# raineyeh/Marching-Cube-for-Implicit-Surfaces

Measured on NVIDIA B200. Metric: Gvoxels/s, higher is better.
Workload: dtype f32

## Files before the change

marching-cube-for-implicit-surfaces_b200/csrc/mcb_api.cu:

```cuda
#include <cuda_runtime.h>
#include <dlfcn.h>

#include <algorithm>
#include <chrono>
#include <future>
#include <cmath>
#include <cstdio>
#include <cstring>
#include <map>
#include <mutex>
#include <new>
#include <string>
#include <vector>

#include "../../include/mcb.h"
#include "mcb_kernels.cuh"
#include "mcb_jit.h"
#include "mcb_lower.h"

using namespace mcbk;

namespace {

struct EqSlot {
// ... 49 lines not shown
    unsigned long long* d_amb = nullptr;
    uint32_t cap_amb = 0;
    size_t cap_tile_entries = 0;
    size_t cap_tiles = 0;
    unsigned long long* d_rec = nullptr;
    uint32_t* d_trioff = nullptr;
    unsigned long long cap_active = 0;
    float4* d_pos = nullptr;
    float4* d_nrm = nullptr;
    unsigned long long cap_tris = 0;
    bool nrm_allocated = false;
    int mesh_mode = MCB_MESH_SOUP;
    float* d_vlist = nullptr;
    float* d_vnrm = nullptr;
    uint32_t* d_tlist = nullptr;
    unsigned long long cap_verts = 0, cap_itris = 0;
    bool vnrm_allocated = false;
    float* h_out_v = nullptr;
    uint32_t* h_out_t = nullptr;
    float* h_out_n = nullptr;
    unsigned long long h_cap_v = 0, h_cap_t = 0;
    cudaStream_t copy_stream = nullptr;
    cudaEvent_t seg_ev[9] = {};
    cudaEvent_t fork_ev[2] = {};
    unsigned long long* d_bounds = nullptr;
    unsigned long long* h_bounds = nullptr;
    bool streamed = false;
    bool seed_on = false;
    int jit = MCB_JIT_AUTO;
    std::string jit_note;
    struct JitKernel { cudaLibrary_t lib = nullptr; cudaKernel_t kernel = nullptr, signs = nullptr, fill = nullptr; };
    const JitKernel* jit_cur = nullptr;
    std::map<std::string, JitKernel> jit_cache;
    struct JitBuilt { std::string err; std::vector<char> cubin; float ms = 0.f; };
    std::map<std::string, std::future<JitBuilt>> jit_pending;
    std::map<std::string, std::string> jit_failed;
    bool jit_sync = false;
    bool jit_used = false;
    float ms_compile = 0.f;
    bool repeat_on = false;
    float repeat_step = 0.f;
    uint32_t* d_cw = nullptr;
    size_t cap_cw = 0;
    float seed[3] = {0.f, 0.f, 0.f};
    void* nccl_comm = nullptr;
    int comm_rank = 0, comm_nranks = 1;
    cudaStream_t comm_stream = nullptr;
// ... 412 lines not shown
    return MCB_OK;
}

int mcb_create(int device, mcb_ctx** out) {
    if (!out) return MCB_E_ARG;
    *out = nullptr;
    int ndev = 0;
    if (cudaGetDeviceCount(&ndev) != cudaSuccess || ndev <= 0 || device < 0 || device >= ndev) return MCB_E_NODEVICE;
    mcb_ctx* ctx = new (std::nothrow) mcb_ctx();
    if (!ctx) return MCB_E_NOMEM;
    ctx->device = device;
    auto bail = [&](int code) { mcb_destroy(ctx); return code; };
    if (cudaSetDevice(device) != cudaSuccess) return bail(MCB_E_NODEVICE);
    cudaDeviceProp prop;
    if (cudaGetDeviceProperties(&prop, device) != cudaSuccess) return bail(MCB_E_NODEVICE);
    ctx->sm_count = prop.multiProcessorCount;
    if (cudaStreamCreateWithFlags(&ctx->own_stream, cudaStreamNonBlocking) != cudaSuccess) return bail(MCB_E_CUDA);
    ctx->stream = ctx->own_stream;
    for (auto& e : ctx->ev)
        if (cudaEventCreate(&e) != cudaSuccess) return bail(MCB_E_CUDA);
    if (cudaStreamCreateWithFlags(&ctx->copy_stream, cudaStreamNonBlocking) != cudaSuccess) return bail(MCB_E_CUDA);
    for (auto& e : ctx->seg_ev)
        if (cudaEventCreateWithFlags(&e, cudaEventDisableTiming) != cudaSuccess) return bail(MCB_E_CUDA);
    for (auto& e : ctx->fork_ev)
        if (cudaEventCreateWithFlags(&e, cudaEventDisableTiming) != cudaSuccess) return bail(MCB_E_CUDA);
    if (cudaMalloc((void**)&ctx->d_bounds, 3 * 9 * 8) != cudaSuccess) return bail(MCB_E_NOMEM);
    if (cudaMallocHost((void**)&ctx->h_bounds, 3 * 9 * 8) != cudaSuccess) return bail(MCB_E_NOMEM);
    if (cudaMalloc((void**)&ctx->d_ctr, sizeof(Counters)) != cudaSuccess) return bail(MCB_E_NOMEM);
    if (cudaMallocHost((void**)&ctx->h_ctr, sizeof(Counters)) != cudaSuccess) return bail(MCB_E_NOMEM);
    ClsTables tb;
    int8_t face[256];
    mcb_build_ambiguity_faces(face);
    for (int q = 0; q < 256; q++) {
        tb.tri[q] = MCB_TRI_WORDS[q];
        tb.face[q] = face[q];
        tb.ntri[q] = (uint8_t)mcb_tri_count(MCB_TRI_WORDS[q]);
        tb.emask[q] = 0;
        for (int e = 0; e < 12; e++) tb.emask[q] |= (uint16_t)((((q >> mcb_edge_a(e)) ^ (q >> mcb_edge_b(e))) & 1) << e);
    }
    if (cudaMalloc((void**)&ctx->d_cls, sizeof(ClsTables)) != cudaSuccess) return bail(MCB_E_NOMEM);
    if (cudaMemcpy(ctx->d_cls, &tb, sizeof tb, cudaMemcpyHostToDevice) != cudaSuccess) return bail(MCB_E_CUDA);
    {
        const int stack_bytes = MCB_MAX_STACK * kEvalRows * kEvalThreads * (int)sizeof(float);
        const void* evals[] = {(const void*)eval_field_kernel<true, true>, (const void*)eval_field_kernel<false, true>,
                               (const void*)eval_blocks_kernel<true>,      (const void*)eval_blocks_kernel<false>,
                               (const void*)eval_field_kernel<true, true, true>, (const void*)eval_blocks_kernel<true, true>};
        for (const void* k : evals)
            if (cudaFuncSetAttribute(k, cudaFuncAttributeMaxDynamicSharedMemorySize, stack_bytes) != cudaSuccess) return bail(MCB_E_CUDA);
// ... 10 lines not shown
    if (rc < 0) return bail(rc);
    *out = ctx;
    return MCB_OK;
}

void mcb_destroy(mcb_ctx* ctx) {
    if (!ctx) return;
    cudaSetDevice(ctx->device);
    if (ctx->stream) cudaStreamSynchronize(ctx->stream);
    for (auto& s : ctx->eq) free_slot(s);
    for (auto& kv : ctx->jit_cache) if (kv.second.lib) cudaLibraryUnload(kv.second.lib);
    cudaFree(ctx->d_fflags); cudaFree(ctx->d_flist); cudaFree(ctx->d_cw); cudaFree(ctx->d_bcls); cudaFree(ctx->d_elist); cudaFree(ctx->d_cand); cudaFree(ctx->d_scls); cudaFree(ctx->d_slist);
    cudaFree(ctx->d_bounds_iv); cudaFree(ctx->d_ent); cudaFree(ctx->d_tile_u32); cudaFree(ctx->d_amb);
    cudaFree(ctx->d_cs); cudaFree(ctx->d_F); cudaFree(ctx->d_S); cudaFree(ctx->d_V); cudaFree(ctx->d_tables);
    cudaFree(ctx->d_cls); cudaFree(ctx->d_ctr);
    if (ctx->h_ctr) cudaFreeHost(ctx->h_ctr);
    cudaFree(ctx->d_rec); cudaFree(ctx->d_trioff); cudaFree(ctx->d_pos); cudaFree(ctx->d_nrm);
    cudaFree(ctx->d_vlist); cudaFree(ctx->d_vnrm); cudaFree(ctx->d_tlist); cudaFree(ctx->d_item); cudaFree(ctx->d_vinfo);
    cudaFree(ctx->d_chunk_new); cudaFree(ctx->d_fn); cudaFree(ctx->d_nh_count); cudaFree(ctx->d_nh_start); cudaFree(ctx->d_nh_cursor);
    cudaFree(ctx->d_nh_sums); cudaFree(ctx->d_nh_adj);
    cudaFree(ctx->d_mark); cudaFree(ctx->d_changed); cudaFree(ctx->d_seed_u32); cudaFree(ctx->d_rec2); cudaFree(ctx->d_trioff2);
    for (auto& e : ctx->ev) if (e) cudaEventDestroy(e);
    for (auto& e : ctx->seg_ev) if (e) cudaEventDestroy(e);
    for (auto& e : ctx->fork_ev) if (e) cudaEventDestroy(e);
    if (ctx->copy_stream) cudaStreamDestroy(ctx->copy_stream);
    mcb_comm_finalize(ctx);
    cudaFree(ctx->d_layer_hist);
    cudaFree(ctx->d_bounds);
    if (ctx->h_bounds) cudaFreeHost(ctx->h_bounds);
    if (ctx->own_stream) cudaStreamDestroy(ctx->own_stream);
    delete ctx;
}

const char* mcb_last_error(const mcb_ctx* ctx) { return ctx ? ctx->err.c_str() : "null context"; }

int mcb_set_stream(mcb_ctx* ctx, void* s) {
    int rc = enter(ctx);
    if (rc != MCB_OK) return rc;
    MCB_CK(cudaStreamSynchronize(ctx->stream));
    ctx->stream = s ? (cudaStream_t)s : ctx->own_stream;
    return MCB_OK;
}

int mcb_set_equation(mcb_ctx* ctx, int slot, const char* equation) {
    int rc = enter(ctx);
    if (rc != MCB_OK) return rc;
    if (slot < 0 || slot > 3) return fail(ctx, MCB_E_ARG, "slot must be 0..3");
// ... 367 lines not shown
    ctx->jit_used = false;
    ctx->field_is_sparse = false;
    int rc;
    if (jit_wanted(ctx, eq)) {
        rc = launch_eval_jit();
        if (rc == MCB_OK) ctx->jit_used = true;
        else if (rc == kJitDeferred) ctx->jit_note = "compiling in the background";
        else if (ctx->jit == MCB_JIT_ON) return rc;
        else ctx->jit_note = ctx->err;
    }
    if (!ctx->jit_used) {
        const size_t smem = (size_t)std::max(1, eq.c.grid_fused_depth) * kEvalRows * kEvalThreads * sizeof(float);
        mcb_program launch;
        bool has_pow, has_fn;
        if ((rc = encode_program(launch, has_pow, has_fn, false)) != MCB_OK) return rc;
        if (has_fn) MCB_LAUNCH((eval_field_kernel<true, true, true>), blocks, kEvalThreads, smem, s, launch, g, ctx->d_tables, ctx->d_F, ctx->d_S, rgpp);
        else if (has_pow) MCB_LAUNCH((eval_field_kernel<true, true>), blocks, kEvalThreads, smem, s, launch, g, ctx->d_tables, ctx->d_F, ctx->d_S, rgpp);
        else MCB_LAUNCH((eval_field_kernel<false, true>), blocks, kEvalThreads, smem, s, launch, g, ctx->d_tables, ctx->d_F, ctx->d_S, rgpp);
        launches++;
    }
    return launch_constraints(*this);
}

int Run::ensure_block_buffers(FieldBlocks* fb, BlockDims* bd) {
    bd->nbx = g.P / kFieldBlockX;
    bd->nby = (g.NV + kFieldBlockY - 1) / kFieldBlockY;
    bd->nbz = (g.NZ + kFieldBlockZ - 1) / kFieldBlockZ;
    bd->nsy = (bd->nby + kSuper - 1) / kSuper;
    bd->nsz = (bd->nbz + kSuper - 1) / kSuper;
    bd->nb = std::max(bd->nbx, std::max(bd->nby, bd->nbz));
    bd->spa = eq.max_per_axis;
    bd->WC = (int)cg.WC;
    bd->cjb = (g.M + 3) / 4;
    bd->ckb = (g.ke - g.kb + 3) / 4;
    const size_t nb = (size_t)bd->nbx * bd->nby * bd->nbz;
    if (nb >= (1ull << 32)) return fail(ctx, MCB_E_CAPACITY, "too many field blocks: split the grid into more z-slabs");
    if (ctx->cap_fblocks < nb) {
        cudaFree(ctx->d_fflags); cudaFree(ctx->d_flist); cudaFree(ctx->d_bcls); cudaFree(ctx->d_elist);
        ctx->d_fflags = nullptr; ctx->d_flist = nullptr; ctx->d_bcls = nullptr; ctx->d_elist = nullptr; ctx->cap_fblocks = 0;
        if (cudaMalloc((void**)&ctx->d_fflags, nb + 16) != cudaSuccess || cudaMalloc((void**)&ctx->d_flist, (nb + 16) * sizeof(uint32_t)) != cudaSuccess ||
            cudaMalloc((void**)&ctx->d_bcls, nb + 16) != cudaSuccess || cudaMalloc((void**)&ctx->d_elist, (nb + 16) * sizeof(uint32_t)) != cudaSuccess)
            return fail(ctx, MCB_E_NOMEM, "cudaMalloc of the field-block lists failed");
        MCB_CK(cudaMemsetAsync(ctx->d_fflags, 0, nb + 16, s));
        MCB_CK(cudaMemsetAsync(ctx->d_bcls, 0, nb + 16, s));
        ctx->cap_fblocks = nb;
    }
    int rc;
    if ((rc = ensure(ctx, &ctx->d_bounds_iv, &ctx->cap_bounds_iv, (size_t)2 * 3 * bd->spa * bd->nb)) != MCB_OK) return rc;
    if ((rc = ensure(ctx, &ctx->d_cand, &ctx->cap_cand, (size_t)((bd->WC + 63) / 64) * bd->cjb * bd->ckb)) != MCB_OK) return rc;
    const size_t nsup = (size_t)bd->nbx * bd->nsy * bd->nsz;
    if (ctx->cap_scls < nsup) {
        cudaFree(ctx->d_scls); cudaFree(ctx->d_slist);
        ctx->d_scls = nullptr; ctx->d_slist = nullptr; ctx->cap_scls = 0;
        MCB_CK(cudaMalloc((void**)&ctx->d_scls, nsup));
        MCB_CK(cudaMalloc((void**)&ctx->d_slist, nsup * sizeof(uint32_t)));
        ctx->cap_scls = nsup;
    }
    *fb = FieldBlocks{bd->nbx, bd->nby, bd->nbz, ctx->d_fflags, ctx->d_flist};
    ctx->bd = *bd;
    return MCB_OK;
}

int Run::launch_block_eval(const FieldBlocks& fb, const uint32_t* list, const unsigned* count) {
    const unsigned fill_ctas = (unsigned)ctx->sm_count * 16;
    int rc;
    if (ctx->jit_used && ctx->jit_cur && ctx->jit_cur->fill) {
        struct { float k[MCB_MAX_K]; } consts;
        std::memcpy(consts.k, eq.grid.k, sizeof consts.k);
        Grid garg = g;
        const float* tables = ctx->d_tables;
        float* F = ctx->d_F;
        uint32_t* S = ctx->d_S;
// ... 17 lines not shown
}

int Run::stage_eval_blocks() {
    FieldBlocks fb;
    BlockDims bd;
    int rc = ensure_block_buffers(&fb, &bd);
    if (rc != MCB_OK) return rc;
    if (ctx->poison_field) {
        MCB_CK(cudaMemsetAsync(ctx->d_F, 0xff, (size_t)g.NZ * g.NV * g.P * sizeof(float), s));
        MCB_CK(cudaMemsetAsync(ctx->d_S, 0x5a, (size_t)g.NZ * g.NV * g.WP * sizeof(uint32_t), s));
    }
    ctx->field_is_sparse = true;
    ctx->jit_used = false;
    if (jit_wanted(ctx, eq)) {
        const mcb_ctx::JitKernel* jk = nullptr;
        rc = jit_module(ctx, eq, &jk);
        if (rc == MCB_OK) { ctx->jit_used = true; ctx->jit_cur = jk; }
        else if (rc == kJitDeferred) ctx->jit_note = "compiling in the background";
        else if (ctx->jit == MCB_JIT_ON) return rc;
        else ctx->jit_note = ctx->err;
    }
    const size_t nblocks = (size_t)bd.nbx * bd.nby * bd.nbz;
    const unsigned nsuper = (unsigned)bd.nbx * (unsigned)bd.nsy * (unsigned)bd.nsz;
    cudaStream_t side = ctx->copy_stream;
    MCB_CK(cudaEventRecord(ctx->fork_ev[0], s));
    MCB_CK(cudaStreamWaitEvent(side, ctx->fork_ev[0], 0));
    MCB_CK(cudaMemsetAsync(ctx->d_cand, 0, (size_t)((bd.WC + 63) / 64) * bd.cjb * bd.ckb * 8, side));
    MCB_CK(cudaMemsetAsync(ctx->d_fflags, 0, nblocks, side));
    MCB_CK(cudaMemsetAsync(ctx->d_bcls, 0xFF, nblocks, side));
    MCB_CK(cudaEventRecord(ctx->fork_ev[1], side));
    MCB_LAUNCH((axis_bounds_kernel), dim3((unsigned)((3 * bd.spa * bd.nb + 127) / 128), 2u), 128, 0, s, ctx->d_tables, g, bd, eq.c.n_axis_slots[0],
               eq.c.n_axis_slots[1], eq.c.n_axis_slots[2], ctx->d_bounds_iv);
    MCB_LAUNCH((super_class_kernel), (nsuper + 127) / 128, 128, 0, s, eq.grid, g, bd, ctx->d_bounds_iv, ctx->decide_blocks ? 1 : 0, ctx->d_scls,
               ctx->d_slist, ctx->d_ctr);
    MCB_CK(cudaStreamWaitEvent(s, ctx->fork_ev[1], 0));
    MCB_LAUNCH((block_class_kernel), (unsigned)ctx->sm_count * 8, 256, 0, s, eq.grid, g, bd, ctx->d_bounds_iv, ctx->d_slist, ctx->decide_blocks ? 1 : 0,
               ctx->d_bcls, ctx->d_fflags, ctx->d_elist, ctx->d_cand, ctx->d_ctr);
    MCB_CK(cudaEventRecord(ctx->fork_ev[0], s));
    MCB_CK(cudaStreamWaitEvent(side, ctx->fork_ev[0], 0));
    MCB_LAUNCH((decided_signs_kernel), (unsigned)ctx->sm_count * 8, 256, 0, side, g, bd, ctx->d_elist, ctx->d_ctr, ctx->d_bcls, ctx->d_scls, ctx->d_S);
    MCB_CK(cudaEventRecord(ctx->fork_ev[1], side));
    launches += 4;
    rc = launch_block_eval(fb, ctx->d_elist, &ctx->d_ctr->eval_blocks);
    MCB_CK(cudaStreamWaitEvent(s, ctx->fork_ev[1], 0));
    if (rc != MCB_OK) return rc;
    return launch_constraints(*this);
}

int Run::stage_classify() {
    int rc;
    MCB_CK(cudaMemsetAsync(ctx->d_ctr, 0, kCountersClassifyBytes, s));
    uint32_t* tu = ctx->d_tile_u32;
    const size_t ct = ctx->cap_tiles;
    const bool skip = ctx->field_is_sparse;
    const ClsScratch sc{ctx->d_ent, tu, tu + ct, tu + 2 * ct, tu + 3 * ct, tu + 4 * ct, ctx->d_amb, ctx->cap_amb, cg.tile_rows * cg.WC,
                        skip ? ctx->d_cand : nullptr, (uint32_t)((g.M + 3) / 4), (uint32_t)((cg.WC + 63) / 64)};
    const uint32_t* cw = nullptr;
    if (g.repeat) {
        const unsigned long long items = (unsigned long long)cg.total_rows * cg.WC;
        if ((rc = ensure(ctx, &ctx->d_cw, &ctx->cap_cw, (size_t)items * 8)) != MCB_OK) return rc;
        MCB_LAUNCH((repeat_words_kernel), (unsigned)ctx->sm_count * 8, 256, 0, s, g, ctx->d_F, cg.WC, ctx->d_cw, items);
        launches++;
        cw = ctx->d_cw;
    }
    const bool need_items = want_indexed || ctx->seed_on;
    if (need_items && (rc = ensure_weld_scratch(ctx, g)) != MCB_OK) return rc;
    unsigned long long* items = need_items ? ctx->d_item : nullptr;
    const unsigned amb_ctas = (unsigned)ctx->sm_count * 2;
    const FieldBlocks apron = skip ? FieldBlocks{ctx->bd.nbx, ctx->bd.nby, ctx->bd.nbz, ctx->d_fflags, ctx->d_flist} : FieldBlocks{0, 0, 0, nullptr, nullptr};
#define MCB_CLASSIFY(HAS_V, REPEAT)                                                                                                   \
    do {                                                                                                                              \
        MCB_LAUNCH((classify_kernel<HAS_V, REPEAT>), tiles, kClsThreads, kClsSmemBytes, s, g, ctx->d_cls, ctx->d_S, dV, cg, sc, ctx->d_ctr, cw); \
        MCB_LAUNCH((ambiguity_kernel<REPEAT>), amb_ctas, 128, 0, s, eq.point, g, ctx->d_cs, ctx->d_cls, sc, ctx->d_ctr, ctx->d_F);          \
        MCB_LAUNCH((tile_scan_kernel), 1, 1024, 0, s, sc, tiles, ctx->d_ctr);                                                             \
        MCB_LAUNCH((compact_kernel<REPEAT>), tiles, kClsThreads, 0, s, g, ctx->d_cls, ctx->d_S, dV, cg, sc, ctx->d_rec, ctx->d_trioff,     \
                   ctx->cap_active, items, cw, apron);                                                                                 \
    } while (0)
    if (cw) { if (dV) MCB_CLASSIFY(true, true); else MCB_CLASSIFY(false, true); }
    else { if (dV) MCB_CLASSIFY(true, false); else MCB_CLASSIFY(false, false); }
// ... 743 lines not shown
```

marching-cube-for-implicit-surfaces_b200/csrc/mcb_kernels.cuh:

```cuda
#pragma once

#include <cuda_runtime.h>
#include <stddef.h>
#include <stdint.h>

#include <type_traits>

#include "mcb_bytecode.h"
#include "mcb_interval.h"
#include "mcb_launch.h"
#include "mcb_tables.h"

namespace mcbk {

constexpr int kEvalThreads = 128;
constexpr int kEvalRows = 16;
constexpr int kClsThreads = 256;
constexpr int kEmitCubes = 64;
constexpr int kEmitThreads = 128;
constexpr int kEmitSlots = 512;
constexpr int kEmitBlocksPerSM = 10;

struct Grid {
    int M;
// ... 383 lines not shown
    if (idx >= 3 * bd.spa * bd.nb) return;
    const int b = idx % bd.nb, slot = (idx / bd.nb) % bd.spa, axis = idx / (bd.nb * bd.spa);
    const int ns = axis == 0 ? nsx : axis == 1 ? nsy : nsz;
    const int nbk = axis == 0 ? bd.nbx : axis == 1 ? (level ? bd.nsy : bd.nby) : (level ? bd.nsz : bd.nbz);
    if (slot >= ns || b >= nbk) return;
    const int span = axis == 0 ? kFieldBlockX : (level ? kSuper : 1) * (axis == 1 ? kFieldBlockY : kFieldBlockZ);
    const int count = axis == 0 ? g.P : axis == 1 ? g.NV : g.NZ;
    const int i0 = b * span, i1 = min(i0 + span + 1, count);
    const float* t = tables + ((size_t)axis * bd.spa + slot) * g.P + (axis == 2 ? g.kb : 0);
    float lo = __ldg(t + i0), hi = lo;
    bool ok = mcb_iv_finite(lo) != 0;
    for (int i = i0 + 1; i < i1; i++) {
        const float v = __ldg(t + i);
        ok = ok && mcb_iv_finite(v);
        lo = v < lo ? v : lo;
        hi = v > hi ? v : hi;
    }
    mcb_ival r;
    r.lo = ok ? lo : -INFINITY;
    r.hi = ok ? hi : INFINITY;
    B[(size_t)level * 3 * bd.spa * bd.nb + idx] = r;
}

constexpr uint8_t kClsInherit = 0xFF;
__device__ __forceinline__ int block_class_of(const uint8_t* __restrict__ cls, const uint8_t* __restrict__ scls, const BlockDims& bd,
                                              int bx, int by, int bz) {
    const int c = (int)cls[((size_t)bz * bd.nby + by) * bd.nbx + bx];
    return c != kClsInherit ? c : (int)scls[((size_t)(bz / kSuper) * bd.nsy + by / kSuper) * bd.nbx + bx];
}

__global__ void __launch_bounds__(128)
super_class_kernel(const __grid_constant__ mcb_program prog , const Grid g,
                   const BlockDims bd, const mcb_ival* __restrict__ B, int decide ,
                   uint8_t* __restrict__ scls, uint32_t* __restrict__ slist, Counters* __restrict__ ctr) {
    const unsigned n = (unsigned)bd.nbx * (unsigned)bd.nsy * (unsigned)bd.nsz;
    const unsigned idx = blockIdx.x * blockDim.x + threadIdx.x;
    const int lane = threadIdx.x & 31;
    int c = 0;
    if (idx < n) {
        const int bx = (int)(idx % (unsigned)bd.nbx), sy = (int)(idx / (unsigned)bd.nbx % (unsigned)bd.nsy), sz = (int)(idx / ((unsigned)bd.nbx * (unsigned)bd.nsy));
        if (decide) c = mcb_interval_class(prog.code, prog.n, prog.k, B + (size_t)3 * bd.spa * bd.nb, bd.spa, bd.nb, bx, sy, sz, g.iso, nullptr);
        scls[idx] = (uint8_t)c;
    }
    const bool undecided = idx < n && c == 0;
    const uint32_t m = __ballot_sync(0xffffffffu, undecided);
    if (m == 0u) return;
    unsigned base = 0;
    if (lane == __ffs(m) - 1) base = atomicAdd(&ctr->eval_supers, (unsigned)__popc(m));
    base = __shfl_sync(0xffffffffu, base, __ffs(m) - 1);
    if (undecided) slist[base + __popc(m & ((1u << lane) - 1u))] = idx;
}

__global__ void __launch_bounds__(256)
block_class_kernel(const __grid_constant__ mcb_program prog, const Grid g, const BlockDims bd, const mcb_ival* __restrict__ B,
                   const uint32_t* __restrict__ slist, int decide, uint8_t* __restrict__ cls ,
                   uint8_t* __restrict__ flags , uint32_t* __restrict__ list,
                   unsigned long long* __restrict__ cand ,
                   Counters* __restrict__ ctr) {
    const unsigned nsuper = ctr->eval_supers;
    const int lane = threadIdx.x & 31;
    const unsigned stride = gridDim.x * blockDim.x;
    const unsigned npad = (nsuper + 31u) & ~31u, total = npad * 16u;
    const int cmw = (bd.WC + 63) / 64;
    for (unsigned t = blockIdx.x * blockDim.x + threadIdx.x; t < total; t += stride) {
        const unsigned sub = t / npad, si = t - sub * npad;
        bool undecided = false;
        int bx = 0, by = 0, bz = 0;
        if (si < nsuper) {
            const unsigned sidx = slist[si];
            bx = (int)(sidx % (unsigned)bd.nbx);
            by = (int)(sidx / (unsigned)bd.nbx % (unsigned)bd.nsy) * kSuper + (int)(sub & 3u);
            bz = (int)(sidx / ((unsigned)bd.nbx * (unsigned)bd.nsy)) * kSuper + (int)(sub >> 2);
            if (by < bd.nby && bz < bd.nbz) {
                const int c = decide ? mcb_interval_class(prog.code, prog.n, prog.k, B, bd.spa, bd.nb, bx, by, bz, g.iso, nullptr) : 0;
                const size_t id = ((size_t)bz * bd.nby + by) * bd.nbx + bx;
                cls[id] = (uint8_t)c;
                undecided = c == 0;
                if (undecided) flags[id] = 2;
            }
        }
        const uint32_t m = __ballot_sync(0xffffffffu, undecided);
        if (m == 0u) continue;
        unsigned base = 0;
        if (lane == __ffs(m) - 1) base = atomicAdd(&ctr->eval_blocks, (unsigned)__popc(m));
        base = __shfl_sync(0xffffffffu, base, __ffs(m) - 1);
        if (!undecided) continue;
        list[base + __popc(m & ((1u << lane) - 1u))] = pack_block(bx, by, bz);
#pragma unroll
        for (int d = 0; d < 4; d++) {
            const int jb = by - (d & 1), kq = bz - (d >> 1);
            if (jb < 0 || kq < 0 || jb >= bd.cjb || kq >= bd.ckb) continue;
            unsigned long long* row = cand + ((size_t)kq * bd.cjb + jb) * cmw;
            if (bx < bd.WC && !((*(volatile unsigned long long*)(row + (bx >> 6)) >> (bx & 63)) & 1ull)) atomicOr(row + (bx >> 6), 1ull << (bx & 63));
            if (bx >= 1 && bx - 1 < bd.WC && !((*(volatile unsigned long long*)(row + ((bx - 1) >> 6)) >> ((bx - 1) & 63)) & 1ull))
                atomicOr(row + ((bx - 1) >> 6), 1ull << ((bx - 1) & 63));
        }
    }
}

__device__ __forceinline__ void write_decided_signs(const Grid& g, uint32_t* __restrict__ S, int bx, int by, int bz, int c, int lane16) {
    const int y = by * kFieldBlockY + (lane16 >> 2), pz = bz * kFieldBlockZ + (lane16 & 3);
    if (y < g.NV && pz < g.NZ) S[((size_t)pz * g.NV + y) * g.WP + bx] = (c & 3) == 2 ? 0xffffffffu : 0u;
}
__global__ void __launch_bounds__(256)
decided_signs_kernel(const Grid g, const BlockDims bd, const uint32_t* __restrict__ list, const Counters* __restrict__ ctr,
                     uint8_t* __restrict__ cls, const uint8_t* __restrict__ scls, uint32_t* __restrict__ S) {
    const unsigned n = ctr->eval_blocks;
    const int lane = threadIdx.x & 31;
    const unsigned nwarps = gridDim.x * (blockDim.x >> 5);
    for (unsigned b = blockIdx.x * (blockDim.x >> 5) + (threadIdx.x >> 5); b < n; b += nwarps) {
        const uint32_t id = list[b];
        const int bx = (int)(id & 0xFFu) + lane % 3 - 1, by = (int)((id >> 8) & 0xFFFu) + (lane / 3) % 3 - 1, bz = (int)(id >> 20) + lane / 9 - 1;
        int c = 0;
        if (lane < 27 && lane != 13 && bx >= 0 && by >= 0 && bz >= 0 && bx < bd.nbx && by < bd.nby && bz < bd.nbz) {
            const size_t bid = ((size_t)bz * bd.nby + by) * bd.nbx + bx;
            unsigned* word = reinterpret_cast<unsigned*>(cls + (bid & ~(size_t)3));
            const unsigned sh = (unsigned)(bid & 3) * 8u;
            for (;;) {
                const unsigned w = *(volatile unsigned*)word, b8 = (w >> sh) & 0xFFu;
                const int cur = b8 == kClsInherit ? (int)scls[((size_t)(bz / kSuper) * bd.nsy + by / kSuper) * bd.nbx + bx] : (int)b8;
                if (cur == 0 || (b8 != kClsInherit && (b8 & 4u))) { c = 0; break; }
                if (atomicCAS(word, w, (w & ~(0xFFu << sh)) | ((unsigned)(cur | 4) << sh)) == w) { c = cur; break; }
            }
        }
        uint32_t todo = __ballot_sync(0xffffffffu, c != 0);
        while (todo) {
            const int src = __ffs(todo) - 1;
            todo &= todo - 1;
            const int nx = __shfl_sync(0xffffffffu, bx, src), ny = __shfl_sync(0xffffffffu, by, src), nz = __shfl_sync(0xffffffffu, bz, src);
            const int nc = __shfl_sync(0xffffffffu, c, src);
            if (lane < 16) write_decided_signs(g, S, nx, ny, nz, nc, lane);
        }
    }
}
__global__ void __launch_bounds__(256)
add_index_base_kernel(uint32_t* __restrict__ tri_list, unsigned long long n, uint32_t delta) {
    const unsigned long long stride = (unsigned long long)gridDim.x * blockDim.x;
    for (unsigned long long q = (unsigned long long)blockIdx.x * blockDim.x + threadIdx.x; q < n; q += stride) tri_list[q] += delta;
}

__global__ void __launch_bounds__(256)
decided_signs_all_kernel(const Grid g, const BlockDims bd, uint8_t* __restrict__ cls, const uint8_t* __restrict__ scls, uint32_t* __restrict__ S) {
    const unsigned nblocks = (unsigned)bd.nbx * (unsigned)bd.nby * (unsigned)bd.nbz;
    const unsigned idx = blockIdx.x * blockDim.x + threadIdx.x;
    if (idx >= nblocks) return;
    const int bx = (int)(idx % (unsigned)bd.nbx), by = (int)(idx / (unsigned)bd.nbx % (unsigned)bd.nby), bz = (int)(idx / ((unsigned)bd.nbx * (unsigned)bd.nby));
    const int c = block_class_of(cls, scls, bd, bx, by, bz);
    if (c == 0 || (c & 4)) return;
    cls[idx] = (uint8_t)(c | 4);
#pragma unroll
    for (int l = 0; l < 16; l++) write_decided_signs(g, S, bx, by, bz, c, l);
}

__global__ void __launch_bounds__(256)
eval_constraint_kernel(const __grid_constant__ mcb_program prog, const Grid g, const float* __restrict__ cs,
                       int op, float rhs, int first, uint32_t* __restrict__ V, long long total_words) {
    const int lane = threadIdx.x & 31;
    const long long widx = (long long)blockIdx.x * 8 + (threadIdx.x >> 5);
    if (widx >= total_words) return;
    const int w = (int)(widx % g.WP);
    const long long row = widx / g.WP;
    const int y = (int)(row % g.NV);
    const int pz = (int)(row / g.NV);
    const int x = w * 32 + lane;
    bool ok = false;
    if (x < g.NV) {
        float v = mcb_interp_scalar(prog.code, prog.n, prog.k, g.sx * cs[x], g.sy * cs[y], g.sz * cs[pz + g.kb],
                                    nullptr, nullptr, nullptr);
        ok = op == 0 ? v > rhs : op == 1 ? v < rhs : op == 2 ? v >= rhs : v <= rhs;
    }
    unsigned bits = __ballot_sync(0xffffffffu, ok);
    if (lane == 0) V[widx] = first ? bits : (V[widx] & bits);
}

constexpr int kClsWarps = kClsThreads / 32;
constexpr int kClsItemCap = 8192;
constexpr int kClsChunkCap = kClsItemCap / 32;
constexpr size_t kClsSmemBytes = (size_t)kClsChunkCap * 4 + (size_t)kClsItemCap * 2;

struct ClsGeom {
    uint32_t WC;
    uint32_t total_rows;
    uint32_t tile_rows;
    uint32_t nstrips;
    uint32_t strip_rows;
    uint32_t inv_wc;
    uint32_t inv_m;
};
__device__ __forceinline__ uint32_t div_small(uint32_t n, uint32_t inv) { return inv ? __umulhi(n, inv) : n; }

struct ClsTables {
    uint64_t tri[256];
    int8_t face[256];
    uint8_t ntri[256];
    uint16_t emask[256];
};

__device__ __forceinline__ void vertex_row_words(const uint32_t* __restrict__ B, uint32_t idx, uint32_t plane, uint32_t r[4]) {
    const uint32_t* p0 = B + idx;
    const uint32_t* p1 = B + (idx + plane);
    const uint32_t a0 = __ldg(p0), a1 = __ldg(p0 + 1);
    const uint32_t b0 = __ldg(p1), b1 = __ldg(p1 + 1);
    r[0] = __funnelshift_r(a0, a1, 1); r[1] = __funnelshift_r(a0, a1, 2);
    r[2] = __funnelshift_r(b0, b1, 1); r[3] = __funnelshift_r(b0, b1, 2);
}
__device__ __forceinline__ void corner_words(const uint32_t lo[4], const uint32_t hi[4], uint32_t c[8]) {
    c[0] = lo[0]; c[1] = lo[1]; c[4] = lo[2]; c[5] = lo[3];
    c[3] = hi[0]; c[2] = hi[1]; c[7] = hi[2]; c[6] = hi[3];
}

__device__ __forceinline__ int code_of(const uint32_t c[8], int b) {
    int code = 0;
#pragma unroll
    for (int v = 0; v < 8; v++) code |= ((c[v] >> b) & 1u) << v;
    return code;
}

__device__ __noinline__ bool ambiguity_redirects(const mcb_program& prog, const Grid& g, const float* __restrict__ cs,
                                                 int face, int i, int j, int k, float iso) {
    float mx = 0.f, my = 0.f, mz = 0.f;
#pragma unroll
    for (int q = 0; q < 4; q++) {
        const int ofs = mcb_corner_ofs(mcb_face_corner(face, q));
        mx += cs[i + 1 + (ofs & 1)];
        my += cs[j + 1 + ((ofs >> 1) & 1)];
        mz += cs[k + 1 + ((ofs >> 2) & 1)];
    }
// ... 34 lines not shown
         item += (unsigned long long)gridDim.x * (blockDim.x >> 5)) {
        const uint32_t w = (uint32_t)(item % WC);
        const unsigned long long row = item / WC;
        const int j = (int)(row % (unsigned)g.M), kz = (int)(row / (unsigned)g.M), i = (int)w * 32 + lane;
        const bool in = i < g.M;
        float iso = 0.f;
        const float* f0 = F + (size_t)(kz + 1) * planep + (size_t)(j + 1) * rowp + (i + 1);
        if (in) iso = cube_iso(g, F, i, j, kz + g.kb);
        uint32_t mine = 0;
#pragma unroll
        for (int v = 0; v < 8; v++) {
            const int o = mcb_corner_ofs(v);
            const bool up = in && __ldg(f0 + (size_t)(o >> 2) * planep + (size_t)((o >> 1) & 1) * rowp + (o & 1)) > iso;
            const uint32_t word = __ballot_sync(0xffffffffu, up);
            if (lane == v) mine = word;
        }
        if (lane < 8) Cw[item * 8 + lane] = mine;
    }
}

template <bool REPEAT>
__device__ __forceinline__ void view_item(ItemView& it, uint32_t item_local, uint32_t j0, uint32_t kz0, const ClsGeom& q,
                                          const Grid& g, const uint32_t* __restrict__ S, const uint32_t* __restrict__ V,
                                          uint32_t plane, const uint32_t* __restrict__ Cw) {
    const uint32_t r = div_small(item_local, q.inv_wc);
    it.w = item_local - r * q.WC;
    const uint32_t jj = j0 + r, dk = div_small(jj, q.inv_m);
    it.j = jj - dk * (uint32_t)g.M;
    it.kz = kz0 + dk;
    const uint32_t idx = ((it.kz + 1u) * (uint32_t)g.NV + (it.j + 1u)) * (uint32_t)g.WP + it.w;
    if (REPEAT) repeat_item_words(Cw, ((size_t)it.kz * (uint32_t)g.M + it.j) * q.WC + it.w, it.c);
    else {
        uint32_t lo[4], hi[4];
        vertex_row_words(S, idx, plane, lo);
        vertex_row_words(S, idx + (uint32_t)g.WP, plane, hi);
        corner_words(lo, hi, it.c);
    }
    it.m = active_mask(it.c, column_mask(g, it.w));
    if (V != nullptr && it.m) it.m &= valid_mask(V, idx, (uint32_t)g.WP, plane);
}

struct ClsScratch {
    unsigned long long* ent;
    uint32_t* nz;
    uint32_t* tile_a;
    uint32_t* tile_t;
    uint32_t* base_a;
    uint32_t* base_t;
    unsigned long long* amb;
    uint32_t cap_amb;
    uint32_t tile_items;
    const unsigned long long* cand;
    uint32_t cjb;
    uint32_t cmw;
};
#define MCB_ENT_NA(e) ((uint32_t)(e) & 63u)
#define MCB_ENT_NT(e) (((uint32_t)(e) >> 6) & 255u)
#define MCB_ENT_ITEM(e) (((uint32_t)(e) >> 14) & 8191u)
#define MCB_ENT_RED(e) ((uint32_t)((e) >> 32))

template <bool HAS_V, bool REPEAT >
__global__ void __launch_bounds__(kClsThreads, 4)
classify_kernel(const Grid g, const ClsTables* __restrict__ gtb, const uint32_t* __restrict__ S, const uint32_t* __restrict__ V,
                const ClsGeom q, const ClsScratch sc, Counters* __restrict__ ctr,
                const uint32_t* __restrict__ Cw ) {
    MCB_DYNAMIC_SMEM(uint32_t, cls_smem);
    uint32_t* bitmap = cls_smem;
    uint16_t* list = reinterpret_cast<uint16_t*>(cls_smem + kClsChunkCap);
    __shared__ uint32_t warp_x[kClsWarps], warp_y[kClsWarps];
    __shared__ uint32_t ncand_s;

    for (int i = threadIdx.x; i < kClsChunkCap; i += kClsThreads) bitmap[i] = 0u;
    __syncthreads();
    const uint32_t tile = blockIdx.x;
    const int lane = threadIdx.x & 31, warp = threadIdx.x >> 5;
    const uint32_t WP = (uint32_t)g.WP, plane = (uint32_t)g.NV * WP, M = (uint32_t)g.M;
    const uint32_t row0 = tile * q.tile_rows;
    const uint32_t rows = min(q.tile_rows, q.total_rows - row0);
    const uint32_t kz0 = row0 / M, j0 = row0 - kz0 * M;

    {
        const uint32_t cjb = sc.cjb;
        const uint32_t r_last = row0 + rows - 1u, kz1 = r_last / M, j1 = r_last - kz1 * M;
        const uint32_t G0 = kz0 * cjb + (j0 >> 2), G1 = kz1 * cjb + (j1 >> 2);
        const uint32_t ncell = (G1 - G0 + 1u) * q.WC;
// ... 33 lines not shown
        }
        for (uint32_t q2 = threadIdx.x; q2 < ncand; q2 += kClsThreads) {
            const uint32_t c = mapped ? (uint32_t)cells[q2] : q2;
            const uint32_t gq = div_small(c, q.inv_wc), w = c - gq * q.WC, G = G0 + gq, kz = G / cjb, jb = G - kz * cjb;
            uint32_t R_lo = kz * M + 4u * jb, R_hi = kz * M + min(4u * jb + 4u, M);
            R_lo = max(R_lo, row0); R_hi = min(R_hi, row0 + rows);
            if (R_lo >= R_hi) continue;
            const uint32_t n = R_hi - R_lo, j = R_lo - kz * M;
            const uint32_t colmask = column_mask(g, w);
            uint32_t item = (R_lo - row0) * q.WC + w;
            uint32_t idx = ((kz + 1u) * (uint32_t)g.NV + (j + 1u)) * WP + w;
            if (REPEAT) {
                for (uint32_t t = 0; t < n; t++) {
                    uint32_t cw8[8];
                    repeat_item_words(Cw, ((size_t)kz * M + (j + t)) * q.WC + w, cw8);
                    uint32_t m = active_mask(cw8, colmask);
                    if (HAS_V && m) m &= valid_mask(V, idx, WP, plane);
                    if (m) atomicOr(&bitmap[item >> 5], 1u << (item & 31u));
                    idx += WP;
                    item += q.WC;
                }
                continue;
            }
            uint32_t lo[4];
            vertex_row_words(S, idx, plane, lo);
            uint32_t any_lo = lo[0] | lo[1] | lo[2] | lo[3], all_lo = lo[0] & lo[1] & lo[2] & lo[3];
#pragma unroll 4
            for (uint32_t t = 0; t < n; t++) {
                uint32_t hi[4];
                vertex_row_words(S, idx + WP, plane, hi);
                const uint32_t any_hi = hi[0] | hi[1] | hi[2] | hi[3], all_hi = hi[0] & hi[1] & hi[2] & hi[3];
                uint32_t m = (any_lo | any_hi) & ~(all_lo & all_hi) & colmask;
                if (HAS_V && m) m &= valid_mask(V, idx, WP, plane);
                if (m) atomicOr(&bitmap[item >> 5], 1u << (item & 31u));
                any_lo = any_hi; all_lo = all_hi;
                idx += WP;
                item += q.WC;
            }
        }
    }
    __syncthreads();

    uint32_t nz;
    {
        constexpr int kPer = (kClsChunkCap + kClsThreads - 1) / kClsThreads;
        uint32_t wd[kPer], mine = 0;
#pragma unroll
        for (int i = 0; i < kPer; i++) {
            const int wi = threadIdx.x * kPer + i;
            wd[i] = wi < kClsChunkCap ? bitmap[wi] : 0u;
            mine += __popc(wd[i]);
        }
        uint32_t inc = mine;
// ... 8 lines not shown
#pragma unroll
        for (int i = 0; i < kPer; i++) {
            uint32_t b = wd[i];
            while (b) {
                const int bit = __ffs(b) - 1;
                b &= b - 1;
                list[base++] = (uint16_t)((threadIdx.x * kPer + i) * 32 + bit);
            }
        }
    }
    __syncthreads();
    if (nz == 0) {
        if (threadIdx.x == 0) { sc.nz[tile] = 0; sc.tile_a[tile] = 0; sc.tile_t[tile] = 0; }
        return;
    }

    unsigned long long* gent = sc.ent + (size_t)tile * sc.tile_items;
    uint32_t sum_a = 0, sum_t = 0;
    for (uint32_t kb = (uint32_t)warp * 32u; kb < nz; kb += kClsThreads) {
        const uint32_t k = kb + (uint32_t)lane;
        if (k < nz) {
            const uint32_t item_local = list[k];
            ItemView it;
            view_item<REPEAT>(it, item_local, j0, kz0, q, g, S, V, plane, Cw);
            const uint32_t na = __popc(it.m);
            uint32_t nt = 0, mm = it.m;
            while (mm) {
                const int b = __ffs(mm) - 1;
                mm &= mm - 1;
                const int code = code_of(it.c, b);
                const int face = (int)(int8_t)__ldg((const signed char*)gtb->face + code);
                if (face >= 0) {
                    const uint32_t slot = atomicAdd(&ctr->amb_n, 1u);
                    if (slot < sc.cap_amb) {
                        sc.amb[2 * (size_t)slot] = ((unsigned long long)tile * sc.tile_items + k) | ((unsigned long long)b << 40) |
                                                   ((unsigned long long)face << 45) | ((unsigned long long)code << 48);
                        sc.amb[2 * (size_t)slot + 1] = (unsigned long long)(it.w * 32 + b) | ((unsigned long long)it.j << 12) |
                                                       ((unsigned long long)(it.kz + g.kb) << 24);
                    }
                }
                nt += __ldg(gtb->ntri + code);
            }
            gent[k] = (unsigned long long)(na | (nt << 6) | (item_local << 14));
            sum_a += na; sum_t += nt;
        }
    }
#pragma unroll
// ... 129 lines not shown
        for (int i = 0; i < kPer; i++) {
            const uint32_t c = threadIdx.x * kPer + i;
            if (c < nchunks) { chunk_a[c] = ba; chunk_t[c] = bt; }
            ba += a[i]; bt += t[i];
        }
    }
    __syncthreads();

    const uint32_t WP = (uint32_t)g.WP, plane = (uint32_t)g.NV * WP, M = (uint32_t)g.M;
    const uint32_t kz0 = row0 / M, j0 = row0 - kz0 * M;
    const unsigned long long tile_a = sc.base_a[tile], tile_t = sc.base_t[tile];
    for (uint32_t kb = (uint32_t)warp * 32u; kb < nz; kb += kClsThreads) {
        const uint32_t k = kb + (uint32_t)lane;
        const unsigned long long e = k < nz ? gent[k] : 0ull;
        const uint32_t mine = MCB_ENT_NA(e) | (MCB_ENT_NT(e) << 16);
        uint32_t inc = mine;
#pragma unroll
        for (int d = 1; d < 32; d <<= 1) { const uint32_t u = __shfl_up_sync(0xffffffffu, inc, d); if (lane >= d) inc += u; }
        if (k >= nz) continue;
        unsigned long long oa = tile_a + chunk_a[kb >> 5] + ((inc - mine) & 0xffffu);
        unsigned long long ot = tile_t + chunk_t[kb >> 5] + ((inc - mine) >> 16);
        ItemView it;
        const uint32_t item_local = MCB_ENT_ITEM(e), red = MCB_ENT_RED(e);
        view_item<REPEAT>(it, item_local, j0, kz0, q, g, S, V, plane, Cw);
        uint32_t m = it.m;
        if (item_info != nullptr)
            item_info[(size_t)tile * sc.tile_items + item_local] = (oa & 0xFFFFFFFFull) | ((unsigned long long)m << 32);
        if (fb.flags != nullptr) {
            const int bx0 = (int)it.w, bx1 = (m >> 29) ? min((int)it.w + 1, fb.nbx - 1) : (int)it.w;
            const int by0 = (int)it.j >> 2, by1 = ((int)it.j + 3) >> 2, bz0 = (int)it.kz >> 2, bz1 = ((int)it.kz + 3) >> 2;
            for (int bz = bz0; bz <= bz1; bz++)
                for (int by = by0; by <= by1; by++)
                    for (int bx = bx0; bx <= bx1; bx++) {
                        uint8_t* f = fb.flags + ((size_t)bz * fb.nby + by) * fb.nbx + bx;
                        if (*f == 0) *f = 1;
                    }
        }
        while (m) {
            const int b = __ffs(m) - 1;
            m &= m - 1;
            const int code = code_of(it.c, b);
            const int tidx = ((red >> b) & 1u) ? 255 - code : code;
            if (oa < cap_active) {
                rec[oa] = (unsigned long long)(it.w * 32 + b) | ((unsigned long long)it.j << 12) |
                          ((unsigned long long)(it.kz + g.kb) << 24) | ((unsigned long long)code << 36) |
                          ((unsigned long long)tidx << 44);
                trioff[oa] = (uint32_t)ot;
// ... 1090 lines not shown
```

Measured before the change: 2149.

## Derive decided-block signs on the fly instead of writing them to the sign grid

Removes the decided_signs pass that wrote constant sign words into S for the neighbours of evaluated blocks. The classify and emit paths now look up block and super-block classes and substitute all-zero or all-one words for decided blocks. The side-stream memsets and fork events are also dropped, with the flag and candidate clears folded into super_class_kernel. classify_kernel's launch-bounds minimum blocks goes from 4 to 5. In exchange, every item view does extra class-table loads and the register pressure may rise.

```diff
diff --git a/marching-cube-for-implicit-surfaces_b200/csrc/mcb_api.cu b/marching-cube-for-implicit-surfaces_b200/csrc/mcb_api.cu
--- a/marching-cube-for-implicit-surfaces_b200/csrc/mcb_api.cu
+++ b/marching-cube-for-implicit-surfaces_b200/csrc/mcb_api.cu
@@ -95,7 +95,6 @@
     unsigned long long h_cap_v = 0, h_cap_t = 0;
     cudaStream_t copy_stream = nullptr;
     cudaEvent_t seg_ev[9] = {};
-    cudaEvent_t fork_ev[2] = {};
     unsigned long long* d_bounds = nullptr;
     unsigned long long* h_bounds = nullptr;
     bool streamed = false;
@@ -554,8 +553,6 @@
     if (cudaStreamCreateWithFlags(&ctx->copy_stream, cudaStreamNonBlocking) != cudaSuccess) return bail(MCB_E_CUDA);
     for (auto& e : ctx->seg_ev)
         if (cudaEventCreateWithFlags(&e, cudaEventDisableTiming) != cudaSuccess) return bail(MCB_E_CUDA);
-    for (auto& e : ctx->fork_ev)
-        if (cudaEventCreateWithFlags(&e, cudaEventDisableTiming) != cudaSuccess) return bail(MCB_E_CUDA);
     if (cudaMalloc((void**)&ctx->d_bounds, 3 * 9 * 8) != cudaSuccess) return bail(MCB_E_NOMEM);
     if (cudaMallocHost((void**)&ctx->h_bounds, 3 * 9 * 8) != cudaSuccess) return bail(MCB_E_NOMEM);
     if (cudaMalloc((void**)&ctx->d_ctr, sizeof(Counters)) != cudaSuccess) return bail(MCB_E_NOMEM);
@@ -612,7 +609,6 @@
     cudaFree(ctx->d_mark); cudaFree(ctx->d_changed); cudaFree(ctx->d_seed_u32); cudaFree(ctx->d_rec2); cudaFree(ctx->d_trioff2);
     for (auto& e : ctx->ev) if (e) cudaEventDestroy(e);
     for (auto& e : ctx->seg_ev) if (e) cudaEventDestroy(e);
-    for (auto& e : ctx->fork_ev) if (e) cudaEventDestroy(e);
     if (ctx->copy_stream) cudaStreamDestroy(ctx->copy_stream);
     mcb_comm_finalize(ctx);
     cudaFree(ctx->d_layer_hist);
@@ -1026,6 +1022,8 @@
     return launch_constraints(*this);
 }
 
+static size_t cand_words(const BlockDims& bd) { return (size_t)((bd.WC + 63) / 64) * bd.cjb * bd.ckb; }
+
 int Run::ensure_block_buffers(FieldBlocks* fb, BlockDims* bd) {
     bd->nbx = g.P / kFieldBlockX;
     bd->nby = (g.NV + kFieldBlockY - 1) / kFieldBlockY;
@@ -1046,12 +1044,11 @@
             cudaMalloc((void**)&ctx->d_bcls, nb + 16) != cudaSuccess || cudaMalloc((void**)&ctx->d_elist, (nb + 16) * sizeof(uint32_t)) != cudaSuccess)
             return fail(ctx, MCB_E_NOMEM, "cudaMalloc of the field-block lists failed");
         MCB_CK(cudaMemsetAsync(ctx->d_fflags, 0, nb + 16, s));
-        MCB_CK(cudaMemsetAsync(ctx->d_bcls, 0, nb + 16, s));
         ctx->cap_fblocks = nb;
     }
     int rc;
     if ((rc = ensure(ctx, &ctx->d_bounds_iv, &ctx->cap_bounds_iv, (size_t)2 * 3 * bd->spa * bd->nb)) != MCB_OK) return rc;
-    if ((rc = ensure(ctx, &ctx->d_cand, &ctx->cap_cand, (size_t)((bd->WC + 63) / 64) * bd->cjb * bd->ckb)) != MCB_OK) return rc;
+    if ((rc = ensure(ctx, &ctx->d_cand, &ctx->cap_cand, (cand_words(*bd) + 1) & ~(size_t)1)) != MCB_OK) return rc;
     const size_t nsup = (size_t)bd->nbx * bd->nsy * bd->nsz;
     if (ctx->cap_scls < nsup) {
         cudaFree(ctx->d_scls); cudaFree(ctx->d_slist);
@@ -1115,27 +1112,15 @@
     }
     const size_t nblocks = (size_t)bd.nbx * bd.nby * bd.nbz;
     const unsigned nsuper = (unsigned)bd.nbx * (unsigned)bd.nsy * (unsigned)bd.nsz;
-    cudaStream_t side = ctx->copy_stream;
-    MCB_CK(cudaEventRecord(ctx->fork_ev[0], s));
-    MCB_CK(cudaStreamWaitEvent(side, ctx->fork_ev[0], 0));
-    MCB_CK(cudaMemsetAsync(ctx->d_cand, 0, (size_t)((bd.WC + 63) / 64) * bd.cjb * bd.ckb * 8, side));
-    MCB_CK(cudaMemsetAsync(ctx->d_fflags, 0, nblocks, side));
-    MCB_CK(cudaMemsetAsync(ctx->d_bcls, 0xFF, nblocks, side));
-    MCB_CK(cudaEventRecord(ctx->fork_ev[1], side));
     MCB_LAUNCH((axis_bounds_kernel), dim3((unsigned)((3 * bd.spa * bd.nb + 127) / 128), 2u), 128, 0, s, ctx->d_tables, g, bd, eq.c.n_axis_slots[0],
                eq.c.n_axis_slots[1], eq.c.n_axis_slots[2], ctx->d_bounds_iv);
     MCB_LAUNCH((super_class_kernel), (nsuper + 127) / 128, 128, 0, s, eq.grid, g, bd, ctx->d_bounds_iv, ctx->decide_blocks ? 1 : 0, ctx->d_scls,
-               ctx->d_slist, ctx->d_ctr);
-    MCB_CK(cudaStreamWaitEvent(s, ctx->fork_ev[1], 0));
+               ctx->d_slist, ctx->d_ctr, reinterpret_cast<uint4*>(ctx->d_fflags), (unsigned)((nblocks + 15) / 16),
+               reinterpret_cast<uint4*>(ctx->d_cand), (unsigned)((cand_words(bd) + 1) / 2));
     MCB_LAUNCH((block_class_kernel), (unsigned)ctx->sm_count * 8, 256, 0, s, eq.grid, g, bd, ctx->d_bounds_iv, ctx->d_slist, ctx->decide_blocks ? 1 : 0,
                ctx->d_bcls, ctx->d_fflags, ctx->d_elist, ctx->d_cand, ctx->d_ctr);
-    MCB_CK(cudaEventRecord(ctx->fork_ev[0], s));
-    MCB_CK(cudaStreamWaitEvent(side, ctx->fork_ev[0], 0));
-    MCB_LAUNCH((decided_signs_kernel), (unsigned)ctx->sm_count * 8, 256, 0, side, g, bd, ctx->d_elist, ctx->d_ctr, ctx->d_bcls, ctx->d_scls, ctx->d_S);
-    MCB_CK(cudaEventRecord(ctx->fork_ev[1], side));
-    launches += 4;
+    launches += 3;
     rc = launch_block_eval(fb, ctx->d_elist, &ctx->d_ctr->eval_blocks);
-    MCB_CK(cudaStreamWaitEvent(s, ctx->fork_ev[1], 0));
     if (rc != MCB_OK) return rc;
     return launch_constraints(*this);
 }
@@ -1147,7 +1132,8 @@
     const size_t ct = ctx->cap_tiles;
     const bool skip = ctx->field_is_sparse;
     const ClsScratch sc{ctx->d_ent, tu, tu + ct, tu + 2 * ct, tu + 3 * ct, tu + 4 * ct, ctx->d_amb, ctx->cap_amb, cg.tile_rows * cg.WC,
-                        skip ? ctx->d_cand : nullptr, (uint32_t)((g.M + 3) / 4), (uint32_t)((cg.WC + 63) / 64)};
+                        skip ? ctx->d_cand : nullptr, (uint32_t)((g.M + 3) / 4), (uint32_t)((cg.WC + 63) / 64),
+                        BlockClasses{skip ? ctx->d_bcls : nullptr, ctx->d_scls, ctx->bd}};
     const uint32_t* cw = nullptr;
     if (g.repeat) {
         const unsigned long long items = (unsigned long long)cg.total_rows * cg.WC;
diff --git a/marching-cube-for-implicit-surfaces_b200/csrc/mcb_kernels.cuh b/marching-cube-for-implicit-surfaces_b200/csrc/mcb_kernels.cuh
--- a/marching-cube-for-implicit-surfaces_b200/csrc/mcb_kernels.cuh
+++ b/marching-cube-for-implicit-surfaces_b200/csrc/mcb_kernels.cuh
@@ -429,20 +429,23 @@
     B[(size_t)level * 3 * bd.spa * bd.nb + idx] = r;
 }
 
-constexpr uint8_t kClsInherit = 0xFF;
 __device__ __forceinline__ int block_class_of(const uint8_t* __restrict__ cls, const uint8_t* __restrict__ scls, const BlockDims& bd,
                                               int bx, int by, int bz) {
-    const int c = (int)cls[((size_t)bz * bd.nby + by) * bd.nbx + bx];
-    return c != kClsInherit ? c : (int)scls[((size_t)(bz / kSuper) * bd.nsy + by / kSuper) * bd.nbx + bx];
+    const int s = (int)__ldg(scls + ((size_t)(bz / kSuper) * bd.nsy + by / kSuper) * bd.nbx + bx);
+    const int c = (int)__ldg(cls + ((size_t)bz * bd.nby + by) * bd.nbx + bx);
+    return s != 0 ? s : c;
 }
 
 __global__ void __launch_bounds__(128)
 super_class_kernel(const __grid_constant__ mcb_program prog , const Grid g,
                    const BlockDims bd, const mcb_ival* __restrict__ B, int decide ,
-                   uint8_t* __restrict__ scls, uint32_t* __restrict__ slist, Counters* __restrict__ ctr) {
+                   uint8_t* __restrict__ scls, uint32_t* __restrict__ slist, Counters* __restrict__ ctr,
+                   uint4* __restrict__ flags, unsigned nflags16, uint4* __restrict__ cand, unsigned ncand16) {
     const unsigned n = (unsigned)bd.nbx * (unsigned)bd.nsy * (unsigned)bd.nsz;
     const unsigned idx = blockIdx.x * blockDim.x + threadIdx.x;
     const int lane = threadIdx.x & 31;
+    for (unsigned i = idx; i < nflags16; i += gridDim.x * blockDim.x) flags[i] = make_uint4(0u, 0u, 0u, 0u);
+    for (unsigned i = idx; i < ncand16; i += gridDim.x * blockDim.x) cand[i] = make_uint4(0u, 0u, 0u, 0u);
     int c = 0;
     if (idx < n) {
         const int bx = (int)(idx % (unsigned)bd.nbx), sy = (int)(idx / (unsigned)bd.nbx % (unsigned)bd.nsy), sz = (int)(idx / ((unsigned)bd.nbx * (unsigned)bd.nsy));
@@ -460,7 +463,7 @@
 
 __global__ void __launch_bounds__(256)
 block_class_kernel(const __grid_constant__ mcb_program prog, const Grid g, const BlockDims bd, const mcb_ival* __restrict__ B,
-                   const uint32_t* __restrict__ slist, int decide, uint8_t* __restrict__ cls ,
+                   const uint32_t* __restrict__ slist, int decide, uint8_t* __restrict__ cls,
                    uint8_t* __restrict__ flags , uint32_t* __restrict__ list,
                    unsigned long long* __restrict__ cand ,
                    Counters* __restrict__ ctr) {
@@ -505,41 +508,6 @@
     }
 }
 
-__device__ __forceinline__ void write_decided_signs(const Grid& g, uint32_t* __restrict__ S, int bx, int by, int bz, int c, int lane16) {
-    const int y = by * kFieldBlockY + (lane16 >> 2), pz = bz * kFieldBlockZ + (lane16 & 3);
-    if (y < g.NV && pz < g.NZ) S[((size_t)pz * g.NV + y) * g.WP + bx] = (c & 3) == 2 ? 0xffffffffu : 0u;
-}
-__global__ void __launch_bounds__(256)
-decided_signs_kernel(const Grid g, const BlockDims bd, const uint32_t* __restrict__ list, const Counters* __restrict__ ctr,
-                     uint8_t* __restrict__ cls, const uint8_t* __restrict__ scls, uint32_t* __restrict__ S) {
-    const unsigned n = ctr->eval_blocks;
-    const int lane = threadIdx.x & 31;
-    const unsigned nwarps = gridDim.x * (blockDim.x >> 5);
-    for (unsigned b = blockIdx.x * (blockDim.x >> 5) + (threadIdx.x >> 5); b < n; b += nwarps) {
-        const uint32_t id = list[b];
-        const int bx = (int)(id & 0xFFu) + lane % 3 - 1, by = (int)((id >> 8) & 0xFFFu) + (lane / 3) % 3 - 1, bz = (int)(id >> 20) + lane / 9 - 1;
-        int c = 0;
-        if (lane < 27 && lane != 13 && bx >= 0 && by >= 0 && bz >= 0 && bx < bd.nbx && by < bd.nby && bz < bd.nbz) {
-            const size_t bid = ((size_t)bz * bd.nby + by) * bd.nbx + bx;
-            unsigned* word = reinterpret_cast<unsigned*>(cls + (bid & ~(size_t)3));
-            const unsigned sh = (unsigned)(bid & 3) * 8u;
-            for (;;) {
-                const unsigned w = *(volatile unsigned*)word, b8 = (w >> sh) & 0xFFu;
-                const int cur = b8 == kClsInherit ? (int)scls[((size_t)(bz / kSuper) * bd.nsy + by / kSuper) * bd.nbx + bx] : (int)b8;
-                if (cur == 0 || (b8 != kClsInherit && (b8 & 4u))) { c = 0; break; }
-                if (atomicCAS(word, w, (w & ~(0xFFu << sh)) | ((unsigned)(cur | 4) << sh)) == w) { c = cur; break; }
-            }
-        }
-        uint32_t todo = __ballot_sync(0xffffffffu, c != 0);
-        while (todo) {
-            const int src = __ffs(todo) - 1;
-            todo &= todo - 1;
-            const int nx = __shfl_sync(0xffffffffu, bx, src), ny = __shfl_sync(0xffffffffu, by, src), nz = __shfl_sync(0xffffffffu, bz, src);
-            const int nc = __shfl_sync(0xffffffffu, c, src);
-            if (lane < 16) write_decided_signs(g, S, nx, ny, nz, nc, lane);
-        }
-    }
-}
 __global__ void __launch_bounds__(256)
 add_index_base_kernel(uint32_t* __restrict__ tri_list, unsigned long long n, uint32_t delta) {
     const unsigned long long stride = (unsigned long long)gridDim.x * blockDim.x;
@@ -547,16 +515,18 @@
 }
 
 __global__ void __launch_bounds__(256)
-decided_signs_all_kernel(const Grid g, const BlockDims bd, uint8_t* __restrict__ cls, const uint8_t* __restrict__ scls, uint32_t* __restrict__ S) {
+decided_signs_all_kernel(const Grid g, const BlockDims bd, const uint8_t* __restrict__ cls, const uint8_t* __restrict__ scls, uint32_t* __restrict__ S) {
     const unsigned nblocks = (unsigned)bd.nbx * (unsigned)bd.nby * (unsigned)bd.nbz;
     const unsigned idx = blockIdx.x * blockDim.x + threadIdx.x;
     if (idx >= nblocks) return;
     const int bx = (int)(idx % (unsigned)bd.nbx), by = (int)(idx / (unsigned)bd.nbx % (unsigned)bd.nby), bz = (int)(idx / ((unsigned)bd.nbx * (unsigned)bd.nby));
     const int c = block_class_of(cls, scls, bd, bx, by, bz);
-    if (c == 0 || (c & 4)) return;
-    cls[idx] = (uint8_t)(c | 4);
-#pragma unroll
-    for (int l = 0; l < 16; l++) write_decided_signs(g, S, bx, by, bz, c, l);
+    if (c == 0) return;
+#pragma unroll
+    for (int l = 0; l < 16; l++) {
+        const int y = by * kFieldBlockY + (l >> 2), pz = bz * kFieldBlockZ + (l & 3);
+        if (y < g.NV && pz < g.NZ) S[((size_t)pz * g.NV + y) * g.WP + bx] = c == 2 ? 0xffffffffu : 0u;
+    }
 }
 
 __global__ void __launch_bounds__(256)
@@ -603,13 +573,35 @@
     uint16_t emask[256];
 };
 
-__device__ __forceinline__ void vertex_row_words(const uint32_t* __restrict__ B, uint32_t idx, uint32_t plane, uint32_t r[4]) {
-    const uint32_t* p0 = B + idx;
-    const uint32_t* p1 = B + (idx + plane);
-    const uint32_t a0 = __ldg(p0), a1 = __ldg(p0 + 1);
-    const uint32_t b0 = __ldg(p1), b1 = __ldg(p1 + 1);
+struct BlockSigns { uint32_t und, one; };
+struct BlockClasses {
+    const uint8_t* cls;
+    const uint8_t* scls;
+    BlockDims bd;
+};
+__device__ __forceinline__ BlockSigns block_signs(const BlockClasses& bc, int bx0, int by0, int bz0, bool y1 ,
+                                                  bool z1 ) {
+    BlockSigns r{0u, 0u};
+#pragma unroll
+    for (int b = 0; b < 8; b++) {
+        if ((((b >> 1) & 1) && !y1) || ((b >> 2) && !z1)) continue;
+        const int bx = min(bx0 + (b & 1), bc.bd.nbx - 1), by = by0 + ((b >> 1) & 1), bz = bz0 + (b >> 2);
+        const int c = block_class_of(bc.cls, bc.scls, bc.bd, bx, by, bz);
+        r.und |= (uint32_t)(c == 0) << b;
+        r.one |= (uint32_t)(c == 2) << b;
+    }
+    return r;
+}
+__device__ __forceinline__ uint32_t sign_word(const uint32_t* __restrict__ B, uint32_t i, const BlockSigns& bs, uint32_t b) {
+    const uint32_t v = __ldg(B + i);
+    return ((bs.und >> b) & 1u) ? v : 0u - ((bs.one >> b) & 1u);
+}
+__device__ __forceinline__ void vertex_row_words(const uint32_t* __restrict__ B, uint32_t idx, uint32_t plane, uint32_t r[4],
+                                                 const BlockSigns& bs = BlockSigns{0xffu, 0u}, uint32_t b0 = 0u, uint32_t b1 = 0u) {
+    const uint32_t a0 = sign_word(B, idx, bs, b0), a1 = sign_word(B, idx + 1u, bs, b0 | 1u);
+    const uint32_t c0 = sign_word(B, idx + plane, bs, b1), c1 = sign_word(B, idx + plane + 1u, bs, b1 | 1u);
     r[0] = __funnelshift_r(a0, a1, 1); r[1] = __funnelshift_r(a0, a1, 2);
-    r[2] = __funnelshift_r(b0, b1, 1); r[3] = __funnelshift_r(b0, b1, 2);
+    r[2] = __funnelshift_r(c0, c1, 1); r[3] = __funnelshift_r(c0, c1, 2);
 }
 __device__ __forceinline__ void corner_words(const uint32_t lo[4], const uint32_t hi[4], uint32_t c[8]) {
     c[0] = lo[0]; c[1] = lo[1]; c[4] = lo[2]; c[5] = lo[3];
@@ -690,7 +682,7 @@
 template <bool REPEAT>
 __device__ __forceinline__ void view_item(ItemView& it, uint32_t item_local, uint32_t j0, uint32_t kz0, const ClsGeom& q,
                                           const Grid& g, const uint32_t* __restrict__ S, const uint32_t* __restrict__ V,
-                                          uint32_t plane, const uint32_t* __restrict__ Cw) {
+                                          uint32_t plane, const uint32_t* __restrict__ Cw, const BlockClasses& bc) {
     const uint32_t r = div_small(item_local, q.inv_wc);
     it.w = item_local - r * q.WC;
     const uint32_t jj = j0 + r, dk = div_small(jj, q.inv_m);
@@ -699,9 +691,12 @@
     const uint32_t idx = ((it.kz + 1u) * (uint32_t)g.NV + (it.j + 1u)) * (uint32_t)g.WP + it.w;
     if (REPEAT) repeat_item_words(Cw, ((size_t)it.kz * (uint32_t)g.M + it.j) * q.WC + it.w, it.c);
     else {
+        const uint32_t dy = (((it.j + 2u) >> 2) - ((it.j + 1u) >> 2)) << 1, dz = (((it.kz + 2u) >> 2) - ((it.kz + 1u) >> 2)) << 2;
+        BlockSigns bs{0xffu, 0u};
+        if (bc.cls != nullptr) bs = block_signs(bc, (int)it.w, (int)(it.j + 1u) >> 2, (int)(it.kz + 1u) >> 2, dy != 0u, dz != 0u);
         uint32_t lo[4], hi[4];
-        vertex_row_words(S, idx, plane, lo);
-        vertex_row_words(S, idx + (uint32_t)g.WP, plane, hi);
+        vertex_row_words(S, idx, plane, lo, bs, 0u, dz);
+        vertex_row_words(S, idx + (uint32_t)g.WP, plane, hi, bs, dy, dy | dz);
         corner_words(lo, hi, it.c);
     }
     it.m = active_mask(it.c, column_mask(g, it.w));
@@ -721,6 +716,7 @@
     const unsigned long long* cand;
     uint32_t cjb;
     uint32_t cmw;
+    BlockClasses blk;
 };
 #define MCB_ENT_NA(e) ((uint32_t)(e) & 63u)
 #define MCB_ENT_NT(e) (((uint32_t)(e) >> 6) & 255u)
@@ -728,7 +724,7 @@
 #define MCB_ENT_RED(e) ((uint32_t)((e) >> 32))
 
 template <bool HAS_V, bool REPEAT >
-__global__ void __launch_bounds__(kClsThreads, 4)
+__global__ void __launch_bounds__(kClsThreads, 5)
 classify_kernel(const Grid g, const ClsTables* __restrict__ gtb, const uint32_t* __restrict__ S, const uint32_t* __restrict__ V,
                 const ClsGeom q, const ClsScratch sc, Counters* __restrict__ ctr,
                 const uint32_t* __restrict__ Cw ) {
@@ -808,13 +804,17 @@
                 }
                 continue;
             }
+            BlockSigns bs{0xffu, 0u};
+            const uint32_t by0 = (j + 1u) >> 2, dz = (((kz + 2u) >> 2) - ((kz + 1u) >> 2)) << 2;
+            if (sc.blk.cls != nullptr) bs = block_signs(sc.blk, (int)w, (int)by0, (int)(kz + 1u) >> 2, ((j + 1u + n) >> 2) != by0, dz != 0u);
             uint32_t lo[4];
-            vertex_row_words(S, idx, plane, lo);
+            vertex_row_words(S, idx, plane, lo, bs, 0u, dz);
             uint32_t any_lo = lo[0] | lo[1] | lo[2] | lo[3], all_lo = lo[0] & lo[1] & lo[2] & lo[3];
 #pragma unroll 4
             for (uint32_t t = 0; t < n; t++) {
+                const uint32_t dy = (((j + 2u + t) >> 2) - by0) << 1;
                 uint32_t hi[4];
-                vertex_row_words(S, idx + WP, plane, hi);
+                vertex_row_words(S, idx + WP, plane, hi, bs, dy, dy | dz);
                 const uint32_t any_hi = hi[0] | hi[1] | hi[2] | hi[3], all_hi = hi[0] & hi[1] & hi[2] & hi[3];
                 uint32_t m = (any_lo | any_hi) & ~(all_lo & all_hi) & colmask;
                 if (HAS_V && m) m &= valid_mask(V, idx, WP, plane);
@@ -869,7 +869,7 @@
         if (k < nz) {
             const uint32_t item_local = list[k];
             ItemView it;
-            view_item<REPEAT>(it, item_local, j0, kz0, q, g, S, V, plane, Cw);
+            view_item<REPEAT>(it, item_local, j0, kz0, q, g, S, V, plane, Cw, sc.blk);
             const uint32_t na = __popc(it.m);
             uint32_t nt = 0, mm = it.m;
             while (mm) {
@@ -1045,7 +1045,7 @@
         unsigned long long ot = tile_t + chunk_t[kb >> 5] + ((inc - mine) >> 16);
         ItemView it;
         const uint32_t item_local = MCB_ENT_ITEM(e), red = MCB_ENT_RED(e);
-        view_item<REPEAT>(it, item_local, j0, kz0, q, g, S, V, plane, Cw);
+        view_item<REPEAT>(it, item_local, j0, kz0, q, g, S, V, plane, Cw, sc.blk);
         uint32_t m = it.m;
         if (item_info != nullptr)
             item_info[(size_t)tile * sc.tile_items + item_local] = (oa & 0xFFFFFFFFull) | ((unsigned long long)m << 32);
```

Measured after the change: 2249 (median of 6 runs). +4.6%, better.
